# ytchen0323/cloud-scale-bwamem

Hardware: AMD Instinct MI355X
Metric: pair-end 2x150bp reads aligned/sec (higher is better)
Workload: dtype int32+u16

## Files before the change

### cloud-scale-bwamem_amd/csrc/bpsw_internal.h

```cpp
#pragma once

#include <hip/hip_runtime.h>
#include <stddef.h>
#include <stdint.h>

#include <condition_variable>
#include <cstdlib>
#include <mutex>
#include <string>
#include <vector>

#include "bpsw.h"
#include "bpsw_ext_group.h"
#include "bpsw_ring.h"

struct bpsw_ctx;

#include <hip/hip_ext.h>

namespace bpsw {

struct KernelEvents {
  hipEvent_t start = nullptr, stop = nullptr;
};
#define BPSW_LAUNCH(ev, kernel, grid, block, lds, stream, ...)                                                          \
  do {                                                                                                                   \
    if ((ev).start || (ev).stop) hipExtLaunchKernelGGL(kernel, grid, block, lds, stream, (ev).start, (ev).stop, 0, __VA_ARGS__); \
    else hipLaunchKernelGGL(kernel, grid, block, lds, stream, __VA_ARGS__);                                               \
  } while (0)


struct MatRows {
  unsigned long long row[5];
};
MatRows pack_mat(const int8_t mat[25]);
// ... 320 lines not shown
  std::mutex mu;
  DeviceBuffer buf;
  long long l_pac = 0;
  DeviceBuffer ann;
  std::vector<long long> ann_off;
  std::vector<int32_t> ann_len;
  std::vector<std::string> ann_name;
};
DeviceRef& device_ref(int device);

struct StreamLease {
  int device;
  hipStream_t s;
  bool pooled;
  bool led = false;
  int slot = -1;
  double wait_ms;
  explicit StreamLease(bpsw_ctx* c, ExtGroupWaiter* w = nullptr, ExtGroupWaiter** members = nullptr, int* n_members = nullptr);
  ~StreamLease();
  StreamLease(const StreamLease&) = delete;
  StreamLease& operator=(const StreamLease&) = delete;
};
struct CopyLane {
  std::mutex mu;
  hipStream_t s = nullptr;
  hipEvent_t ev = nullptr;
};
CopyLane& copy_lane(int device);
double wall_ms();
int ext_group_max();
int ext_group_waiting(int device);
void ext_group_counts(int device, unsigned long long out[3]);
void ext_group_complete(int device, ExtGroupWaiter** members, int n_members, int status, float span_ms);
void ext_call_mark(int device);
double ext_call_age_ms(int device);
double stat_ms();
int sw_launches_in_flight(int device);
void sw_launch_in_flight(int device, int delta);
double wait_est_update(double est, double took_ms, int polls, bool napped);
bool wait_naps(double est_ms);
void wait_nap(double est_ms);
void wait_poll_pause(int polls, double waited_ms, double est_ms);
hipError_t wait_event(bpsw_ctx* c, hipEvent_t ev, int kind);
int zerocopy_mask();
bool spin_wait();
[[nodiscard]] RefHold ref_snapshot(const bpsw_ctx* c, const uint8_t** pac, long long* l_pac);

int finish_pending_ext(bpsw_ctx* c);
int finish_pending_sw(bpsw_ctx* c);
inline int finish_pending(bpsw_ctx* c) {
  const int a = finish_pending_ext(c), b = finish_pending_sw(c);
  return a != BPSW_OK ? a : b;
}

int run_sw_jobs_host(bpsw_ctx* c, const bpsw_opt_t* opt, const bpsw_sw_jobs_t* jobs, int32_t* out);
struct SwStage {
  int n;
  size_t o_qlen, o_tlen, o_qoff, o_toff, o_qrev, o_qpool, o_tpool, o_packed, total, q_pool_bytes, t_pool_bytes;
  uint8_t* base;
};
int sw_stage_begin(bpsw_ctx* c, int n, size_t q_pool_bytes, size_t t_pool_bytes, SwStage* st);
int sw_stage_run(bpsw_ctx* c, const bpsw_opt_t* opt, int xtra, const SwStage& st, int mq, int mt, bool pac_mode, const int32_t** results);

struct ChainDevJob {
  int n_reads;
  const long long* seed_beg;
// ... 40 lines not shown
  bpsw::ExtScoring ext_sc;
  int8_t ext_mat[25];
  bpsw::DeviceBuffer d_wire, d_out, d_pre, d_sw_in, d_sw_out, d_sw_scratch, d_gl_z, d_ext_lists;
  size_t staged_bytes = 0;
  bpsw::DeviceBuffer d_sift;
  bpsw::DeviceBuffer d_seed[5];
  bpsw::DeviceBuffer d_chain;
  struct PendingExt { bool active = false; const void* d_wire = nullptr; size_t wire_bytes = 0; int n_tasks = 0; void* d_out = nullptr;
                      hipStream_t s = nullptr; int qcap = 0, rcap = 0; } pend_ext;
  int ext_geom_q = 0, ext_geom_r = 0;
  struct PendingSw { bool active = false; bpsw_sw_jobs_t jobs; bpsw_opt_t opt; void* d_out = nullptr; hipStream_t s = nullptr;
                     int cap_qlen = 0, cap_tlen = 0;
                     bool verified = false;
  } pend_sw;
  int sw_geom_qlen = 0, sw_geom_tlen = 0;
  float last_tail_ms = 0.f;
  int last_tail_jobs = 0, last_tail_resubmitted = 0;
  double tail_host_ms[3] = {0., 0., 0.};
  bool have_tail_ev = false;

  bpsw::PinnedBuffer h_stage_in, h_stage_out, h_pre;
  int shortcut_mask = 63;
  std::vector<int> ext_long_tasks;
  double wait_est_ms[6] = {0., 0., 0., 0., 0., 0.};
  bool ring_abandoned = false;
  uint32_t ring_seq = 0;
  void* rescue_scratch = nullptr;
  bpsw_stats_t stats;
  float last_ext_ms = 0.f, last_sw_ms = 0.f;
  bool have_ext_ev = false, have_sw_ev = false;
  bpsw::DeviceBuffer d_chain_tab;
};

namespace bpsw {
struct ContextEntry {
  std::unique_lock<std::mutex> lock;
  int rc = BPSW_OK;
  explicit ContextEntry(bpsw_ctx* c) : lock(c->mu) {
    if (c->ring_abandoned) { rc = fail(BPSW_ERR_DEVICE, "this context gave up a ring batch (watchdog / integrity): create a new one"); return; }
    const hipError_t e = hipSetDevice(c->device);
    if (e != hipSuccess) { rc = fail(BPSW_ERR_DEVICE, std::string("hipSetDevice: ") + hipGetErrorString(e)); return; }
    rc = finish_pending(c);
  }
};
}
```

### cloud-scale-bwamem_amd/csrc/bpsw_rescue.cpp

```cpp
#include <stdlib.h>
#include <string.h>

#include <algorithm>
#include <vector>

#include "bpsw_internal.h"
#include "bpsw_klib_sort.h"
#include "bpsw_rescue_skip.h"

using namespace bpsw;

namespace {

typedef bpsw_alnreg_t Reg;

struct LtRe {
  bool operator()(const Reg& x, const Reg& y) const { return x.re < y.re; }
};
struct LtScore {
  bool operator()(const Reg& x, const Reg& y) const {
    return x.score > y.score || (x.score == y.score && (x.rb < y.rb || (x.rb == y.rb && x.qb < y.qb)));
  }
};
struct LtReRb {
  bool operator()(const Reg& x, const Reg& y) const { return x.re < y.re || (x.re == y.re && x.rb < y.rb); }
};


int sort_dedup(std::vector<Reg>& v, float mask, int mode) {
  int n = (int)v.size();
// ... 12 lines not shown
      const int64_t mr = std::min(q.re - q.rb, p.re - p.rb);
      const int64_t mq = std::min<int64_t>(q.qe - q.qb, p.qe - p.qb);
      if ((float)orr > mask * (float)mr && (float)oq > mask * (float)mq) {
        if (p.score < q.score) { p.qe = p.qb; break; }
        q.qe = q.qb;
      }
    }
  }
  int m = 0;
  for (int i = 0; i < n; ++i)
    if (a[i].qe > a[i].qb) a[m++] = a[i];
  n = m;
  if (mode == BPSW_RESCUE_C) klib_order_sort((size_t)n, a, LtScore());
  else insertion_sort(a, a + n, LtScore());
  for (int i = 1; i < n; ++i)
    if (a[i].score == a[i - 1].score && a[i].rb == a[i - 1].rb && a[i].qb == a[i - 1].qb) a[i].qe = a[i].qb;
  m = n < 1 ? 0 : 1;
  for (int i = 1; i < n; ++i)
    if (a[i].qe > a[i].qb) a[m++] = a[i];
  v.resize((size_t)m);
  return m;
}

inline int infer_dir(int64_t l_pac, int64_t b1, int64_t b2, int64_t* dist) { return rescue_infer_dir(l_pac, b1, b2, dist); }

struct Want { int64_t x; int32_t mate; };
struct Scratch {
  std::vector<int64_t> t_base;
  std::vector<int64_t> job_x;
  std::vector<size_t> job_round;
  std::vector<int32_t> results;
  std::vector<uint8_t> used;
  std::vector<Want> want, want_next;
  std::vector<int32_t> touched;
  std::vector<int64_t> mate_slot;
  std::vector<int32_t> staged_mates;
  std::vector<Reg> arena;
  std::vector<int64_t> fin_off;
  std::vector<int32_t> fin_cnt;
  std::vector<uint8_t> done;
  std::vector<Reg> anchors[2], v[2];
};

struct Group {
  const bpsw_opt_t* opt;
  const bpsw_rescue_group_t* g;
  int mode;
  bool pac_mode;
  Scratch* S;
  int failed_mask;
  int32_t pes_low[4], pes_high[4];
};

void skip_flags(const Group& G, const Reg& a, const Reg* mates, size_t n_mates, int skip[4]) {
  rescue_skip_flags(G.g->l_pac, G.pes_low, G.pes_high, G.failed_mask, G.mode == BPSW_RESCUE_SCALA, a.rb, mates ? &mates->rb : nullptr, sizeof(Reg), n_mates, skip);
}

inline int64_t win_len(const Group& G, int64_t x) {
  if (!G.pac_mode) return G.g->ref_len[x];
  int64_t b = G.g->ref_rb[x], e = G.g->ref_re[x];
  if (b < 0 && e < 0) return 0;
  if (e < b) std::swap(b, e);
  if (e > (G.g->l_pac << 1)) e = G.g->l_pac << 1;
  if (b < 0) b = 0;
  if (!(b >= G.g->l_pac || e <= G.g->l_pac)) return 0;
  return e - b > 0 ? e - b : 0;
}
inline bool window_ok(const Group& G, int64_t x) { return win_len(G, x) == G.g->ref_re[x] - G.g->ref_rb[x]; }

bool make_region(const Group& G, const int32_t aln[7], int r, int l_ms, int64_t x, Reg* out) {
  if (!(aln[0] >= G.opt->min_seed_len && aln[6] >= 0)) return false;
  const bool is_rev = (r >> 1) != (r & 1);
  const int64_t l2 = G.g->l_pac << 1, rbeg = G.g->ref_rb[x];
  Reg b;
  memset(&b, 0, sizeof b);
  if (is_rev) {
    b.qb = l_ms - (aln[2] + 1); b.qe = l_ms - aln[6];
    b.rb = l2 - (rbeg + aln[1] + 1); b.re = l2 - (rbeg + aln[5]);
  } else {
    b.qb = aln[6]; b.qe = aln[2] + 1;
    if (G.mode == BPSW_RESCUE_C) { b.rb = rbeg + aln[5]; b.re = rbeg + aln[1] + 1; }
    else { b.rb = rbeg + aln[1] + 1; b.re = rbeg + aln[1] + 1; }
  }
  b.score = aln[0]; b.csub = aln[3]; b.secondary = -1;
  b.seedcov = (int32_t)(std::min<int64_t>(b.re - b.rb, b.qe - b.qb) >> 1);
  *out = b;
  return true;
}

static const int32_t kNoHit[7] = {0, -1, -1, -1, -1, -1, -1};
inline const int32_t* result_of(Group& G, int64_t x, int l_ms) {
// ... 96 lines not shown
                                 int32_t* out_cnt, bpsw_alnreg_t* out_regs, int64_t out_cap, int64_t* out_total) {
  if (!c || !opt || !g || !out_cnt || !out_total) return fail(BPSW_ERR_ARG, "matesw_group: null argument");
  if (mode != BPSW_RESCUE_C && mode != BPSW_RESCUE_SCALA) return fail(BPSW_ERR_ARG, "matesw_group: bad mode");
  const int G_ = g->group_size;
  if (G_ < 0) return fail(BPSW_ERR_ARG, "matesw_group: negative group size");
  ContextEntry entry(c);
  if (entry.rc != BPSW_OK) return entry.rc;

  const double t_begin = stat_ms();
  double t_pack = 0., t_replay = 0.;
  if (!c->rescue_scratch) c->rescue_scratch = new Scratch();
  Scratch& S = *(Scratch*)c->rescue_scratch;
  Group GR;
  GR.opt = opt; GR.g = g; GR.mode = mode; GR.S = &S;
  GR.pac_mode = g->ref_pool == nullptr;
  const bool rescue_on = (opt->flag & 0x20) == 0;

  GR.failed_mask = 0;
  for (int r = 0; r < 4; ++r) { GR.failed_mask |= (g->pes[r].failed ? 1 : 0) << r; GR.pes_low[r] = g->pes[r].low; GR.pes_high[r] = g->pes[r].high; }
  S.t_base.clear();
  S.want.clear(); S.touched.clear();
  int64_t nreg = 0, nref = 0;
  {
    const int32_t* reg_cnt = g->reg_cnt;
    const int32_t* ref_cnt = g->ref_cnt;
    const int32_t* seq_len = g->seq_len;
    const int64_t* seq_off = g->seq_off;
    const uint64_t pool_bytes = g->seq_pool_bytes;
    const int max_matesw = opt->max_matesw, pen_unpaired = opt->pen_unpaired;
    for (int k = 0; k < G_; ++k) {
      const int e0 = 2 * k;
      const int rc[2] = {reg_cnt[e0], reg_cnt[e0 + 1]}, fc[2] = {ref_cnt[e0], ref_cnt[e0 + 1]}, sl[2] = {seq_len[e0], seq_len[e0 + 1]};
      if ((rc[0] | rc[1] | fc[0] | fc[1] | sl[0] | sl[1]) < 0) return fail(BPSW_ERR_ARG, "matesw_group: negative count");
      if ((uint64_t)(seq_off[e0] + sl[0]) > pool_bytes || (uint64_t)(seq_off[e0 + 1] + sl[1]) > pool_bytes)
        return fail(BPSW_ERR_ARG, "matesw_group: mate outside seq_pool");
      const int64_t base[2] = {nreg, nreg + rc[0]}, rowb[2] = {nref, nref + fc[0]};
      nreg += (int64_t)rc[0] + rc[1]; nref += (int64_t)fc[0] + fc[1];
      if (!rescue_on) continue;
      __builtin_prefetch(g->regs + nreg + 12);
      __builtin_prefetch(g->regs + nreg + 13);
#ifndef BPSW_PLAN_PF_ROWS
#define BPSW_PLAN_PF_ROWS 16
#endif
      if (BPSW_PLAN_PF_ROWS > 0) {
        __builtin_prefetch(g->ref_rb + 4 * (nref + BPSW_PLAN_PF_ROWS));
        __builtin_prefetch(g->ref_re + 4 * (nref + BPSW_PLAN_PF_ROWS));
        if (!GR.pac_mode) __builtin_prefetch(g->ref_len + 4 * (nref + BPSW_PLAN_PF_ROWS));
      }
      if (rc[0] == 1 && rc[1] == 1 && fc[0] >= 1 && fc[1] >= 1 && sl[0] >= 1 && sl[1] >= 1 && max_matesw >= 1 && pen_unpaired >= 0) {
        const int64_t rb0 = g->regs[base[0]].rb, rb1 = g->regs[base[1]].rb;
        int64_t d01, d10;
        const int r01 = infer_dir(g->l_pac, rb0, rb1, &d01), r10 = infer_dir(g->l_pac, rb1, rb0, &d10);
        if (mode == BPSW_RESCUE_SCALA) { d01 = (int64_t)(int32_t)d01; d10 = (int64_t)(int32_t)d10; }
        const int m0 = GR.failed_mask | ((d01 >= GR.pes_low[r01] && d01 <= GR.pes_high[r01]) ? 1 << r01 : 0);
        const int m1 = GR.failed_mask | ((d10 >= GR.pes_low[r10] && d10 <= GR.pes_high[r10]) ? 1 << r10 : 0);
        if (m0 == 15 && m1 == 15) continue;
      }
      bool touched = false;
      for (int i = 0; i < 2; ++i) {
        const int mate = e0 + (i ^ 1);
        if (sl[i ^ 1] < 1 || rc[i] == 0 || fc[i] == 0) continue;
        const Reg* init = g->regs + base[i];
        const Reg* minit = g->regs + base[i ^ 1];
        const int n_init = rc[i], n_mate = rc[i ^ 1];
        const int thr = init[0].score - pen_unpaired;
        int j = 0;
        bool emitted = false;
        for (int ai = 0; ai < n_init; ++ai) {
          const Reg& a = init[ai];
          if (!(a.score >= thr)) continue;
          if (j >= max_matesw || j >= fc[i]) break;
          if (emitted) break;
          int skip[4];
          skip_flags(GR, a, minit, (size_t)n_mate, skip);
          if (skip[0] + skip[1] + skip[2] + skip[3] != 4) {
            const int64_t xrow = rowb[i] + j;
            for (int r = 0; r < 4; ++r)
              if (!skip[r] && window_ok(GR, xrow * 4 + r)) { S.want.push_back({xrow * 4 + r, mate}); touched = true; emitted = true; }
          }
          ++j;
        }
      }
      if (touched) {
        S.touched.push_back(k);
        S.t_base.push_back(base[0]); S.t_base.push_back(base[1]); S.t_base.push_back(rowb[0]); S.t_base.push_back(rowb[1]);
      }
    }
  }
  RefHold ref_hold;
  if (GR.pac_mode && nref > 0) {
    const uint8_t* d_pac = nullptr;
    long long loaded = 0;
    ref_hold = ref_snapshot(c, &d_pac, &loaded);
    if (loaded <= 0) return fail(BPSW_ERR_ARG, "matesw_group: ref_pool is null and no reference is loaded (bpsw_ref_load)");
    if (loaded != g->l_pac) return fail(BPSW_ERR_ARG, "matesw_group: l_pac differs from the loaded reference");
  }
  S.job_x.clear(); S.job_round.clear();
  S.results.clear(); S.used.clear();
  const double t_planned = stat_ms();

  const int xtra_base = BPSW_KSW_XSUBO | BPSW_KSW_XSTART | (opt->min_seed_len * opt->a);
  const size_t nt = S.touched.size();
  S.arena.clear();
  S.fin_off.assign(2 * nt, 0); S.fin_cnt.assign(2 * nt, 0); S.done.assign(nt, 0);
  S.mate_slot.assign(2 * (size_t)G_, (int64_t)-1);
  S.staged_mates.clear();
  uint64_t rounds = 0;
  const uint64_t speculated = S.want.size();
  size_t n_done = 0;
  for (;;) {
// ... 145 lines not shown
```

### cloud-scale-bwamem_amd/csrc/bpsw_runtime.cpp

```cpp
#include <stdlib.h>
#include <string.h>

#include <sched.h>
#include <time.h>

#include <algorithm>
#include <atomic>
#include <condition_variable>

#pragma weak launch_ext_group
#include "bpsw_internal.h"

namespace bpsw {

static thread_local std::string g_err;
void set_error(const std::string& msg) { g_err = msg; }
int fail(int code, const std::string& msg) {
  g_err = msg;
  return code;
}

struct RingPauseForFree {
  int dev = 0;
  RingPauseForFree() { if (hipGetDevice(&dev) != hipSuccess) dev = 0; ring_pause(dev); }
  ~RingPauseForFree() { ring_resume(dev); }
};

hipError_t DeviceBuffer::reserve(size_t bytes) {
  if (bytes <= cap) return hipSuccess;
  size_t want = cap ? cap : 1 << 20;
  while (want < bytes) want <<= 1;
  if (ptr) { RingPauseForFree paused; (void)hipFree(ptr); }
  ptr = nullptr;
  cap = 0;
// ... 128 lines not shown
int zerocopy_mask() {
  static const int m = getenv("BPSW_ZEROCOPY") ? atoi(getenv("BPSW_ZEROCOPY")) : 7;
  return m;
}

double wait_est_update(double est, double took_ms, int polls, bool napped) {
  (void)polls; (void)napped;
  if (est <= 0.) return took_ms;
  return 0.75 * est + 0.25 * std::min(took_ms, 3.0 * est + 0.2);
}
bool wait_naps(double est_ms) { return est_ms > 0.15 && est_ms * 700.0 - 60.0 > 20.0; }

void wait_nap(double est_ms) {
  if (est_ms > 0.15) {
    const double nap_us = est_ms * 700.0 - 60.0;
    if (nap_us > 20.0) { timespec ts = {0, (long)(nap_us * 1000.0)}; nanosleep(&ts, nullptr); }
  }
}
void wait_poll_pause(int polls, double waited_ms, double est_ms) {
  if (polls < 64 && waited_ms < est_ms * 1.3 + 0.05) sched_yield();
  else { timespec ts = {0, 20000}; nanosleep(&ts, nullptr); }
}

hipError_t wait_event(bpsw_ctx* c, hipEvent_t ev, int kind) {
  if (spin_wait()) return hipEventSynchronize(ev);
  double& est = c->wait_est_ms[kind & 3];
  const double t0 = wall_ms();
  const bool napped = wait_naps(est);
  wait_nap(est);
  hipError_t e;
  int polls = 0;
  while ((e = hipEventQuery(ev)) == hipErrorNotReady) wait_poll_pause(++polls, wall_ms() - t0, est);
  est = wait_est_update(est, wall_ms() - t0, polls, napped);
  return e;
}

double stat_ms() {
  static const bool cpu = getenv("BPSW_STATS_CLOCK") && getenv("BPSW_STATS_CLOCK")[0] == 'c';
  if (!cpu) return wall_ms();
  timespec ts;
  clock_gettime(CLOCK_THREAD_CPUTIME_ID, &ts);
  return 1e3 * (double)ts.tv_sec + 1e-6 * (double)ts.tv_nsec;
}

double wall_ms() {
  timespec ts;
  clock_gettime(CLOCK_MONOTONIC, &ts);
  return 1e3 * (double)ts.tv_sec + 1e-6 * (double)ts.tv_nsec;
}
// ... 27 lines not shown
  }();
  return cap;
}
int stream_share() {
  static const int n = [] {
    const char* e = getenv("BPSW_STREAM_SHARE");
    const int v = e ? atoi(e) : 1;
    return v < 1 ? 1 : (v > 8 ? 8 : v);
  }();
  return n;
}
}

static std::atomic<long long> g_ext_last_us[64];
void ext_call_mark(int device) { g_ext_last_us[device >= 0 && device < 64 ? device : 0].store((long long)(wall_ms() * 1e3), std::memory_order_relaxed); }
double ext_call_age_ms(int device) {
  const long long t = g_ext_last_us[device >= 0 && device < 64 ? device : 0].load(std::memory_order_relaxed);
  return t == 0 ? 1e12 : wall_ms() - (double)t * 1e-3;
}

CopyLane& copy_lane(int device) {
  static CopyLane table[64];
  return table[device >= 0 && device < 64 ? device : 0];
}

int ext_group_max() {
  static const int n = [] {
    const char* e = getenv("BPSW_EXT_GROUP_MAX");
    const int v = e ? atoi(e) : EXT_GROUP_SLOTS;
    return v < 1 ? 1 : (v > EXT_GROUP_SLOTS ? EXT_GROUP_SLOTS : v);
  }();
  return n;
}
int ext_group_waiting(int device) { return stream_pool(device).q.waiting_compatible(); }
void ext_group_counts(int device, unsigned long long out[3]) { stream_pool(device).q.counts(out); }
void ext_group_complete(int device, ExtGroupWaiter** members, int n_members, int status, float span_ms) {
  stream_pool(device).q.complete(members, n_members, status, span_ms);
}

static int pool_take(StreamPool& P, int cap) {
  if (P.streams.capacity() < 64) { P.streams.reserve(64); P.pending.reserve(64); }
  int best = -1;
  for (size_t k = 0; k < P.streams.size(); ++k)
    if (best < 0 || P.pending[k] < P.pending[(size_t)best]) best = (int)k;
  if (best >= 0 && P.pending[(size_t)best] == 0) { ++P.pending[(size_t)best]; return best; }
  if ((int)P.streams.size() < cap) {
// ... 155 lines not shown
  if (!c) return fail(BPSW_ERR_ARG, "null context");
  std::lock_guard<std::mutex> g(c->mu);
  c->shortcut_mask = mask < 0 ? 63 : (mask & 63);
  apply_shortcuts(c->shortcut_mask, c->ext_mat, &c->ext_sc.exact_a, &c->ext_sc.certify, &c->ext_sc.tail_bound);
  return BPSW_OK;
}

int bpsw_set_ext_scoring(bpsw_ctx_t* c, const int8_t mat[25], int zdrop, int zdrop_mode) {
  if (!c) return fail(BPSW_ERR_ARG, "null context");
  if (zdrop_mode != BPSW_ZDROP_SCALA && zdrop_mode != BPSW_ZDROP_BWA) return fail(BPSW_ERR_ARG, "bad zdrop_mode");
  std::lock_guard<std::mutex> g(c->mu);
  if (mat) memcpy(c->ext_mat, mat, 25);
  c->ext_sc.mat = pack_mat(c->ext_mat);
  c->ext_sc.mat_max = c->ext_mat[0];
  for (int k = 1; k < 25; ++k) c->ext_sc.mat_max = c->ext_mat[k] > c->ext_sc.mat_max ? c->ext_mat[k] : c->ext_sc.mat_max;
  c->ext_sc.zdrop = zdrop;
  c->ext_sc.zdrop_mode = zdrop_mode;
  apply_shortcuts(c->shortcut_mask, c->ext_mat, &c->ext_sc.exact_a, &c->ext_sc.certify, &c->ext_sc.tail_bound);
  return BPSW_OK;
}



static inline int rd16(const uint8_t* b, size_t at) { return (int16_t)(b[at] | (b[at + 1] << 8)); }
static inline int rd32(const uint8_t* b, size_t at) {
  return (int32_t)((uint32_t)b[at] | ((uint32_t)b[at + 1] << 8) | ((uint32_t)b[at + 2] << 16) | ((uint32_t)b[at + 3] << 24));
}

static int scan_wire(const uint8_t* wire, size_t bytes, long long l_pac, int* n_out, int* maxq, int* maxr, bool* coord,
                     std::vector<int>* long_tasks, int* maxr_short, int* n_mid_out) {
  if (!wire || bytes < 32 || (bytes & 3)) return fail(BPSW_ERR_ARG, "extend: wire batch shorter than its header or not word sized");
  const int n = rd32(wire, 8);
  const int fmt = wire[7];
  if (fmt != 0 && fmt != BPSW_WIRE_COORDS) return fail(BPSW_ERR_ARG, "extend: unknown wire format (header byte 7)");
  const bool co = fmt == BPSW_WIRE_COORDS;
  const size_t rec_bytes = co ? 40 : 32;
  if (n < 0 || 32 + rec_bytes * (size_t)n > bytes) return fail(BPSW_ERR_ARG, "extend: task table exceeds the buffer");
  if ((int8_t)wire[0] < 0 || (int8_t)wire[1] < 1 || (int8_t)wire[2] < 0 || (int8_t)wire[3] < 1)
    return fail(BPSW_ERR_ARG, "extend: gap opens must be >= 0 and gap extensions >= 1 (a zero extension divides by zero in SWUtil.scala:110-115)");
  if ((int8_t)wire[6] < 0) return fail(BPSW_ERR_ARG, "extend: negative band width (w travels as a signed byte: at most 127)");
  if (co && l_pac <= 0) return fail(BPSW_ERR_ARG, "extend: a coordinate batch needs the reference on the device (bpsw_ref_load)");
  const int wband = (int8_t)wire[6];
  int mq = 0, mr = 0, mrs = 0;
  const size_t words = bytes >> 2;
  const bool all_long = (int8_t)wire[2] + (int8_t)wire[3] <= 0;
  long_tasks->clear();
  int mid = 0;
  for (int t = 0; t < n; ++t) {
    const size_t at = 32 + rec_bytes * (size_t)t;
    const int lq = rd16(wire, at), lr = rd16(wire, at + 2), rq = rd16(wire, at + 4), rr = rd16(wire, at + 6);
    if (lq < 0 || lr < 0 || rq < 0 || rr < 0) return fail(BPSW_ERR_ARG, "extend: negative sequence length in task table");
    const long long pos = rd32(wire, at + 8);
    const long long w = co ? ((long long)lq + rq + 7) / 8 : ((long long)lq + lr + rq + rr + 7) / 8;
    if (pos < 8 + (long long)(rec_bytes / 4) * n || (unsigned long long)(pos + w) > words)
      return fail(BPSW_ERR_ARG, "extend: task sequence offset outside the buffer");
    if (lq > mq) mq = lq;
    if (rq > mq) mq = rq;
    const bool is_long = all_long || lq > 255 || rq > 255;
    const bool is_mid = !is_long && (lq > 127 || rq > 127);
    if (is_mid) ++mid;
    if (is_long) long_tasks->push_back(t);
    int task_mr = 0;
    if (co) {
      const int len = rd16(wire, at + 18);
      long long rb;
      memcpy(&rb, wire + at + 32, 8);
      if (rb < 0 || rb > (l_pac << 1)) return fail(BPSW_ERR_ARG, "extend: task window outside the reference or bridging its two strands");
      const long long lo = rb - lr, hi = rb + len + rr;
      if (len < 0 || lo < 0 || hi > (l_pac << 1) || (lo < l_pac && hi > l_pac))
        return fail(BPSW_ERR_ARG, "extend: task window outside the reference or bridging its two strands");
      const int sl = std::min(lr, lq + 2 * wband + 2), sr = std::min(rr, rq + 2 * wband + 2);
      task_mr = std::max(sl, sr);
    } else {
      task_mr = std::max(lr, rr);
    }
    if (task_mr > mr) mr = task_mr;
    if (!is_long && task_mr > mrs) mrs = task_mr;
  }
  if (mq > BPSW_EXT_MAX_QLEN || mr > BPSW_EXT_MAX_RLEN) return fail(BPSW_ERR_LIMIT, "extend: sequence longer than the kernel limit");
  *n_out = n; *maxq = mq; *maxr = mr; *coord = co; *maxr_short = mrs; *n_mid_out = mid;
  return BPSW_OK;
}

static int extend_batch_impl(bpsw_ctx_t* c, const uint8_t* wire, size_t wire_bytes, int16_t* out, size_t out_len, uint8_t* side_how,
                             const int16_t** out_view = nullptr);

int bpsw_extend_batch(bpsw_ctx_t* c, const uint8_t* wire, size_t wire_bytes, int16_t* out, size_t out_len) {
  return extend_batch_impl(c, wire, wire_bytes, out, out_len, nullptr);
}

int bpsw_extend_stage(bpsw_ctx_t* c, size_t bytes, uint8_t** buf) {
  if (!c || !buf) return fail(BPSW_ERR_ARG, "extend_stage: null argument");
  ContextEntry entry(c);
  if (entry.rc != BPSW_OK) return entry.rc;
  HIP_TRY(c->h_stage_in.reserve(bytes + bytes / 8 + 4096));
  c->staged_bytes = bytes;
  *buf = (uint8_t*)c->h_stage_in.ptr;
  return BPSW_OK;
}

int bpsw_extend_commit(bpsw_ctx_t* c, size_t wire_bytes, const int16_t** out, size_t* out_len) {
  if (!c || !out) return fail(BPSW_ERR_ARG, "extend_commit: null argument");
  const uint8_t* staged = nullptr;
// ... 114 lines not shown
                                   RingRecords{(uint32_t*)c->h_stage_out.ptr, 5, (size_t)n, 4, "extension"});
      if (run.how == RingRun::failed) {
        if (run.submitted) c->ring_abandoned = true;
        return run.rc;
      }
      if (run.how == RingRun::unwritten) {
        static std::atomic<bool> said{false};
        if (!said.exchange(true)) fprintf(stderr, "bPSW: an extension batch came back from the ring with unwritten records; it is run again through a launch (%s)\n", bpsw_last_error());
      }
      if (run.how == RingRun::done) {
        ring_kernel_ms = run.span_ms;
        t_dev1 = stat_ms();
        via_ring = true;
        c->stats.ext_ring_calls++;
      } else {
        copy_first_ms = 0.;
      }
    }
  }
  if (!via_ring) {
    const bool copy_first = sw_launches_in_flight(c->device) > 0;
    if (copy_first) {
      const double t_c0 = stat_ms();
      CopyLane& L = copy_lane(c->device);
      {
        std::lock_guard<std::mutex> lk(L.mu);
        if (!L.s) HIP_TRY(hipStreamCreateWithFlags(&L.s, hipStreamNonBlocking));
        HIP_TRY(hipMemcpyAsync(c->d_wire.ptr, c->h_stage_in.ptr, stage_bytes, hipMemcpyHostToDevice, L.s));
        HIP_TRY(hipStreamSynchronize(L.s));
      }
      copy_first_ms = stat_ms() - t_c0;
    }
    const bool zc_out = (zerocopy_mask() & 1) != 0;
    int16_t* k_out = zc_out ? (int16_t*)c->h_stage_out.ptr : (int16_t*)c->d_out.ptr;
    int* const d_queue_words = (int*)((char*)c->d_pre.ptr + 128);
    ExtCallItem me;
    memset(&me.gm, 0, sizeof me.gm);
    const bool groupable = &launch_ext_group != nullptr && ext_group_max() > 1 && !coord && use_sift && lazy_full && zc_out && !side_how;
    if (groupable) {
      ExtMember& m = me.gm.m;
      m.wire = (const uint32_t*)c->d_wire.ptr; m.n_tasks = n; m.out = k_out; m.sc = c->ext_sc; m.queue = d_queue_words;
      m.defer = (int*)((char*)c->d_wire.ptr + list_off); m.defer_post = (int*)(k_out + 10 * (size_t)n); m.short_qmax = 255;
      m.sift_flag = (uint8_t*)c->d_sift.ptr; m.sift_recs = (uint4*)((char*)c->d_sift.ptr + sift_rec_off);
      m.todo_count = d_queue_words + 2; m.todo_list = (int*)((char*)c->d_sift.ptr + todo_off);
      m.sift_dm = sift_dm; m.sift_dn = sift_uniform_dn(c->ext_mat, c->ext_sc.exact_a); m.sift_qmax = 127; m.heavy_min = heavy_min;
      me.gm.qcap = std::min(mq, 255); me.gm.rcap = mr_short;
      if (!copy_first) { me.copy_dst = c->d_wire.ptr; me.copy_src = c->h_stage_in.ptr; me.copy_bytes = stage_bytes; }
    }
    ExtGroupWaiter gw;
    gw.compatible = groupable;
    gw.item = &me;
    ExtGroupWaiter* led[EXT_GROUP_SLOTS];
    int n_led = 0;
// ... 280 lines not shown
```

Before: 265.7 million.

## Factor out rescue planning, branchless wire scan, and configurable copy-lane locking

```diff
diff --git a/cloud-scale-bwamem_amd/csrc/bpsw_copy_lane.h b/cloud-scale-bwamem_amd/csrc/bpsw_copy_lane.h
--- /dev/null
+++ b/cloud-scale-bwamem_amd/csrc/bpsw_copy_lane.h
@@ -0,0 +1,62 @@
+#pragma once
+#include <stddef.h>
+
+#include <mutex>
+
+namespace bpsw {
+
+enum CopyLaneMode { COPY_LANE_LOCK = 0, COPY_LANE_FIFO = 1, COPY_LANE_TWO = 2 };
+#ifndef COPY_LANE_DEFAULT
+#define COPY_LANE_DEFAULT COPY_LANE_LOCK
+#endif
+
+inline int copy_lane_mode_of(const char* s, int otherwise) {
+  if (!s) return otherwise;
+  if (s[0] == 'l') return COPY_LANE_LOCK;
+  if (s[0] == 'f') return COPY_LANE_FIFO;
+  if (s[0] == 't') return COPY_LANE_TWO;
+  return otherwise;
+}
+
+struct CopyLaneLocks {
+  std::mutex enqueue;
+  std::mutex head;
+};
+
+template <class Ops, class Wait>
+inline int copy_lane_copy(CopyLaneLocks& L, Ops& ops, int mode, void* dst, const void* src, size_t bytes, typename Ops::Event ev, Wait&& wait) {
+  if (mode == COPY_LANE_FIFO) {
+    {
+      std::lock_guard<std::mutex> lk(L.enqueue);
+      int rc = ops.enqueue_copy(dst, src, bytes);
+      if (rc == 0) rc = ops.record(ev);
+      if (rc != 0) return rc;
+    }
+    return wait(ev);
+  }
+  if (mode == COPY_LANE_TWO) {
+    std::unique_lock<std::mutex> first(L.enqueue);
+    int rc = ops.enqueue_copy(dst, src, bytes);
+    if (rc == 0) rc = ops.record(ev);
+    if (rc != 0) return rc;
+    std::lock_guard<std::mutex> second(L.head);
+    first.unlock();
+    return ops.synchronize(ev, false);
+  }
+  std::lock_guard<std::mutex> lk(L.enqueue);
+  const int rc = ops.enqueue_copy(dst, src, bytes);
+  if (rc != 0) return rc;
+  return ops.synchronize(ev, true);
+}
+
+template <class Ops, class Pause>
+inline int copy_lane_poll(Ops& ops, typename Ops::Event ev, Pause&& pause) {
+  for (;;) {
+    bool done = false;
+    const int rc = ops.query(ev, &done);
+    if (rc != 0 || done) return rc;
+    pause();
+  }
+}
+
+}
diff --git a/cloud-scale-bwamem_amd/csrc/bpsw_internal.h b/cloud-scale-bwamem_amd/csrc/bpsw_internal.h
--- a/cloud-scale-bwamem_amd/csrc/bpsw_internal.h
+++ b/cloud-scale-bwamem_amd/csrc/bpsw_internal.h
@@ -11,6 +11,7 @@
 #include <vector>
 
 #include "bpsw.h"
+#include "bpsw_copy_lane.h"
 #include "bpsw_ext_group.h"
 #include "bpsw_ring.h"
 
@@ -377,11 +378,12 @@
   StreamLease& operator=(const StreamLease&) = delete;
 };
 struct CopyLane {
-  std::mutex mu;
+  CopyLaneLocks locks;
   hipStream_t s = nullptr;
-  hipEvent_t ev = nullptr;
 };
 CopyLane& copy_lane(int device);
+int copy_lane_mode();
+hipError_t copy_lane_h2d(bpsw_ctx* c, void* dst, const void* src, size_t bytes);
 double wall_ms();
 int ext_group_max();
 int ext_group_waiting(int device);
@@ -397,6 +399,7 @@
 void wait_nap(double est_ms);
 void wait_poll_pause(int polls, double waited_ms, double est_ms);
 hipError_t wait_event(bpsw_ctx* c, hipEvent_t ev, int kind);
+hipError_t wait_event_est(hipEvent_t ev, double* est_ms);
 int zerocopy_mask();
 bool spin_wait();
 [[nodiscard]] RefHold ref_snapshot(const bpsw_ctx* c, const uint8_t** pac, long long* l_pac);
@@ -483,7 +486,7 @@
   bpsw::PinnedBuffer h_stage_in, h_stage_out, h_pre;
   int shortcut_mask = 63;
   std::vector<int> ext_long_tasks;
-  double wait_est_ms[6] = {0., 0., 0., 0., 0., 0.};
+  double wait_est_ms[7] = {0., 0., 0., 0., 0., 0., 0.};
   bool ring_abandoned = false;
   uint32_t ring_seq = 0;
   void* rescue_scratch = nullptr;
diff --git a/cloud-scale-bwamem_amd/csrc/bpsw_rescue.cpp b/cloud-scale-bwamem_amd/csrc/bpsw_rescue.cpp
--- a/cloud-scale-bwamem_amd/csrc/bpsw_rescue.cpp
+++ b/cloud-scale-bwamem_amd/csrc/bpsw_rescue.cpp
@@ -6,6 +6,7 @@
 
 #include "bpsw_internal.h"
 #include "bpsw_klib_sort.h"
+#include "bpsw_rescue_plan.h"
 #include "bpsw_rescue_skip.h"
 
 using namespace bpsw;
@@ -64,9 +65,7 @@
   return m;
 }
 
-inline int infer_dir(int64_t l_pac, int64_t b1, int64_t b2, int64_t* dist) { return rescue_infer_dir(l_pac, b1, b2, dist); }
-
-struct Want { int64_t x; int32_t mate; };
+typedef RescueWant Want;
 struct Scratch {
   std::vector<int64_t> t_base;
   std::vector<int64_t> job_x;
@@ -98,17 +97,8 @@
   rescue_skip_flags(G.g->l_pac, G.pes_low, G.pes_high, G.failed_mask, G.mode == BPSW_RESCUE_SCALA, a.rb, mates ? &mates->rb : nullptr, sizeof(Reg), n_mates, skip);
 }
 
-inline int64_t win_len(const Group& G, int64_t x) {
-  if (!G.pac_mode) return G.g->ref_len[x];
-  int64_t b = G.g->ref_rb[x], e = G.g->ref_re[x];
-  if (b < 0 && e < 0) return 0;
-  if (e < b) std::swap(b, e);
-  if (e > (G.g->l_pac << 1)) e = G.g->l_pac << 1;
-  if (b < 0) b = 0;
-  if (!(b >= G.g->l_pac || e <= G.g->l_pac)) return 0;
-  return e - b > 0 ? e - b : 0;
-}
-inline bool window_ok(const Group& G, int64_t x) { return win_len(G, x) == G.g->ref_re[x] - G.g->ref_rb[x]; }
+inline int64_t win_len(const Group& G, int64_t x) { return rescue_win_len(G.g, G.pac_mode, x); }
+inline bool window_ok(const Group& G, int64_t x) { return rescue_window_ok(G.g, G.pac_mode, x); }
 
 bool make_region(const Group& G, const int32_t aln[7], int r, int l_ms, int64_t x, Reg* out) {
   if (!(aln[0] >= G.opt->min_seed_len && aln[6] >= 0)) return false;
@@ -251,70 +241,14 @@
   S.want.clear(); S.touched.clear();
   int64_t nreg = 0, nref = 0;
   {
-    const int32_t* reg_cnt = g->reg_cnt;
-    const int32_t* ref_cnt = g->ref_cnt;
-    const int32_t* seq_len = g->seq_len;
-    const int64_t* seq_off = g->seq_off;
-    const uint64_t pool_bytes = g->seq_pool_bytes;
-    const int max_matesw = opt->max_matesw, pen_unpaired = opt->pen_unpaired;
-    for (int k = 0; k < G_; ++k) {
-      const int e0 = 2 * k;
-      const int rc[2] = {reg_cnt[e0], reg_cnt[e0 + 1]}, fc[2] = {ref_cnt[e0], ref_cnt[e0 + 1]}, sl[2] = {seq_len[e0], seq_len[e0 + 1]};
-      if ((rc[0] | rc[1] | fc[0] | fc[1] | sl[0] | sl[1]) < 0) return fail(BPSW_ERR_ARG, "matesw_group: negative count");
-      if ((uint64_t)(seq_off[e0] + sl[0]) > pool_bytes || (uint64_t)(seq_off[e0 + 1] + sl[1]) > pool_bytes)
-        return fail(BPSW_ERR_ARG, "matesw_group: mate outside seq_pool");
-      const int64_t base[2] = {nreg, nreg + rc[0]}, rowb[2] = {nref, nref + fc[0]};
-      nreg += (int64_t)rc[0] + rc[1]; nref += (int64_t)fc[0] + fc[1];
-      if (!rescue_on) continue;
-      __builtin_prefetch(g->regs + nreg + 12);
-      __builtin_prefetch(g->regs + nreg + 13);
-#ifndef BPSW_PLAN_PF_ROWS
-#define BPSW_PLAN_PF_ROWS 16
-#endif
-      if (BPSW_PLAN_PF_ROWS > 0) {
-        __builtin_prefetch(g->ref_rb + 4 * (nref + BPSW_PLAN_PF_ROWS));
-        __builtin_prefetch(g->ref_re + 4 * (nref + BPSW_PLAN_PF_ROWS));
-        if (!GR.pac_mode) __builtin_prefetch(g->ref_len + 4 * (nref + BPSW_PLAN_PF_ROWS));
-      }
-      if (rc[0] == 1 && rc[1] == 1 && fc[0] >= 1 && fc[1] >= 1 && sl[0] >= 1 && sl[1] >= 1 && max_matesw >= 1 && pen_unpaired >= 0) {
-        const int64_t rb0 = g->regs[base[0]].rb, rb1 = g->regs[base[1]].rb;
-        int64_t d01, d10;
-        const int r01 = infer_dir(g->l_pac, rb0, rb1, &d01), r10 = infer_dir(g->l_pac, rb1, rb0, &d10);
-        if (mode == BPSW_RESCUE_SCALA) { d01 = (int64_t)(int32_t)d01; d10 = (int64_t)(int32_t)d10; }
-        const int m0 = GR.failed_mask | ((d01 >= GR.pes_low[r01] && d01 <= GR.pes_high[r01]) ? 1 << r01 : 0);
-        const int m1 = GR.failed_mask | ((d10 >= GR.pes_low[r10] && d10 <= GR.pes_high[r10]) ? 1 << r10 : 0);
-        if (m0 == 15 && m1 == 15) continue;
-      }
-      bool touched = false;
-      for (int i = 0; i < 2; ++i) {
-        const int mate = e0 + (i ^ 1);
-        if (sl[i ^ 1] < 1 || rc[i] == 0 || fc[i] == 0) continue;
-        const Reg* init = g->regs + base[i];
-        const Reg* minit = g->regs + base[i ^ 1];
-        const int n_init = rc[i], n_mate = rc[i ^ 1];
-        const int thr = init[0].score - pen_unpaired;
-        int j = 0;
-        bool emitted = false;
-        for (int ai = 0; ai < n_init; ++ai) {
-          const Reg& a = init[ai];
-          if (!(a.score >= thr)) continue;
-          if (j >= max_matesw || j >= fc[i]) break;
-          if (emitted) break;
-          int skip[4];
-          skip_flags(GR, a, minit, (size_t)n_mate, skip);
-          if (skip[0] + skip[1] + skip[2] + skip[3] != 4) {
-            const int64_t xrow = rowb[i] + j;
-            for (int r = 0; r < 4; ++r)
-              if (!skip[r] && window_ok(GR, xrow * 4 + r)) { S.want.push_back({xrow * 4 + r, mate}); touched = true; emitted = true; }
-          }
-          ++j;
-        }
-      }
-      if (touched) {
-        S.touched.push_back(k);
-        S.t_base.push_back(base[0]); S.t_base.push_back(base[1]); S.t_base.push_back(rowb[0]); S.t_base.push_back(rowb[1]);
-      }
-    }
+    RescuePlanCfg cfg;
+    cfg.failed_mask = GR.failed_mask;
+    for (int r = 0; r < 4; ++r) { cfg.low[r] = GR.pes_low[r]; cfg.high[r] = GR.pes_high[r]; }
+    cfg.scala = mode == BPSW_RESCUE_SCALA; cfg.pac_mode = GR.pac_mode; cfg.rescue_on = rescue_on;
+    cfg.max_matesw = opt->max_matesw; cfg.pen_unpaired = opt->pen_unpaired;
+    const int prc = rescue_plan(g, cfg, S.want, S.touched, S.t_base, &nreg, &nref);
+    if (prc == RESCUE_PLAN_NEGATIVE_COUNT) return fail(BPSW_ERR_ARG, "matesw_group: negative count");
+    if (prc != RESCUE_PLAN_OK) return fail(BPSW_ERR_ARG, "matesw_group: mate outside seq_pool");
   }
   RefHold ref_hold;
   if (GR.pac_mode && nref > 0) {
diff --git a/cloud-scale-bwamem_amd/csrc/bpsw_rescue_plan.h b/cloud-scale-bwamem_amd/csrc/bpsw_rescue_plan.h
--- /dev/null
+++ b/cloud-scale-bwamem_amd/csrc/bpsw_rescue_plan.h
@@ -0,0 +1,128 @@
+#pragma once
+#include <stdint.h>
+
+#include <utility>
+#include <vector>
+
+#include "bpsw.h"
+#include "bpsw_rescue_skip.h"
+
+namespace bpsw {
+
+struct RescueWant { int64_t x; int32_t mate; };
+
+struct RescuePlanCfg {
+  int failed_mask;
+  int32_t low[4], high[4];
+  bool scala;
+  bool pac_mode;
+  bool rescue_on;
+  int max_matesw, pen_unpaired;
+};
+
+enum { RESCUE_PLAN_OK = 0, RESCUE_PLAN_NEGATIVE_COUNT = 1, RESCUE_PLAN_MATE_OUTSIDE = 2 };
+
+#ifndef RESCUE_PLAN_AHEAD
+#define RESCUE_PLAN_AHEAD 32
+#endif
+
+inline int64_t rescue_win_len(const bpsw_rescue_group_t* g, bool pac_mode, int64_t x) {
+  if (!pac_mode) return g->ref_len[x];
+  int64_t b = g->ref_rb[x], e = g->ref_re[x];
+  if (b < 0 && e < 0) return 0;
+  if (e < b) std::swap(b, e);
+  if (e > (g->l_pac << 1)) e = g->l_pac << 1;
+  if (b < 0) b = 0;
+  if (!(b >= g->l_pac || e <= g->l_pac)) return 0;
+  return e - b > 0 ? e - b : 0;
+}
+inline bool rescue_window_ok(const bpsw_rescue_group_t* g, bool pac_mode, int64_t x) {
+  return rescue_win_len(g, pac_mode, x) == g->ref_re[x] - g->ref_rb[x];
+}
+
+inline void rescue_plan_prefetch(const void* base, int64_t at, size_t elem_bytes) {
+  __builtin_prefetch((const void*)((uintptr_t)base + (uintptr_t)at * elem_bytes));
+}
+
+inline bool rescue_plan_all_skipped(int64_t l_pac, const RescuePlanCfg& cfg, int64_t a_rb, int64_t m_rb) {
+  int64_t d;
+  const int r = rescue_infer_dir(l_pac, a_rb, m_rb, &d);
+  if (cfg.scala) d = (int64_t)(int32_t)d;
+  const int in = (int)(d >= cfg.low[r]) & (int)(d <= cfg.high[r]);
+  return (cfg.failed_mask | (in << r)) == 15;
+}
+
+inline void rescue_plan_walk_pair(const bpsw_rescue_group_t* g, const RescuePlanCfg& cfg, int k, int64_t base0, int64_t rowb0,
+                                  std::vector<RescueWant>& want, std::vector<int32_t>& touched_pairs, std::vector<int64_t>& t_base) {
+  const int e0 = 2 * k;
+  const int rc[2] = {g->reg_cnt[e0], g->reg_cnt[e0 + 1]}, fc[2] = {g->ref_cnt[e0], g->ref_cnt[e0 + 1]}, sl[2] = {g->seq_len[e0], g->seq_len[e0 + 1]};
+  const int64_t base[2] = {base0, base0 + rc[0]}, rowb[2] = {rowb0, rowb0 + fc[0]};
+  bool touched = false;
+  for (int i = 0; i < 2; ++i) {
+    const int mate = e0 + (i ^ 1);
+    if (sl[i ^ 1] < 1 || rc[i] == 0 || fc[i] == 0) continue;
+    const bpsw_alnreg_t* init = g->regs + base[i];
+    const bpsw_alnreg_t* minit = g->regs + base[i ^ 1];
+    const int n_init = rc[i], n_mate = rc[i ^ 1];
+    const int thr = init[0].score - cfg.pen_unpaired;
+    int j = 0;
+    bool emitted = false;
+    for (int ai = 0; ai < n_init; ++ai) {
+      const bpsw_alnreg_t& a = init[ai];
+      if (!(a.score >= thr)) continue;
+      if (j >= cfg.max_matesw || j >= fc[i]) break;
+      if (emitted) break;
+      int skip[4];
+      rescue_skip_flags(g->l_pac, cfg.low, cfg.high, cfg.failed_mask, cfg.scala, a.rb, n_mate ? &minit->rb : nullptr, sizeof(bpsw_alnreg_t),
+                        (size_t)n_mate, skip);
+      if (skip[0] + skip[1] + skip[2] + skip[3] != 4) {
+        const int64_t xrow = rowb[i] + j;
+        for (int r = 0; r < 4; ++r)
+          if (!skip[r] && rescue_window_ok(g, cfg.pac_mode, xrow * 4 + r)) { want.push_back({xrow * 4 + r, mate}); touched = true; emitted = true; }
+      }
+      ++j;
+    }
+  }
+  if (touched) {
+    touched_pairs.push_back(k);
+    t_base.push_back(base[0]); t_base.push_back(base[1]); t_base.push_back(rowb[0]); t_base.push_back(rowb[1]);
+  }
+}
+
+inline int rescue_plan(const bpsw_rescue_group_t* g, const RescuePlanCfg& cfg, std::vector<RescueWant>& want, std::vector<int32_t>& touched,
+                       std::vector<int64_t>& t_base, int64_t* nreg_out, int64_t* nref_out) {
+  const int G = g->group_size;
+  const int32_t* reg_cnt = g->reg_cnt;
+  const int32_t* ref_cnt = g->ref_cnt;
+  const int32_t* seq_len = g->seq_len;
+  const int64_t* seq_off = g->seq_off;
+  const bpsw_alnreg_t* regs = g->regs;
+  const uint64_t pool_bytes = g->seq_pool_bytes;
+  const int64_t l_pac = g->l_pac;
+  const bool fast_shape = cfg.max_matesw >= 1 && cfg.pen_unpaired >= 0;
+  int64_t nreg = 0, nref = 0;
+  int err = RESCUE_PLAN_OK;
+  for (int k = 0; k < G; ++k) {
+    const int e0 = 2 * k;
+    const int rc0 = reg_cnt[e0], rc1 = reg_cnt[e0 + 1], fc0 = ref_cnt[e0], fc1 = ref_cnt[e0 + 1], sl0 = seq_len[e0], sl1 = seq_len[e0 + 1];
+    if ((rc0 | rc1 | fc0 | fc1 | sl0 | sl1) < 0) { err = RESCUE_PLAN_NEGATIVE_COUNT; break; }
+    if ((uint64_t)(seq_off[e0] + sl0) > pool_bytes || (uint64_t)(seq_off[e0 + 1] + sl1) > pool_bytes) { err = RESCUE_PLAN_MATE_OUTSIDE; break; }
+    const int64_t base0 = nreg, rowb0 = nref;
+    nreg += (int64_t)rc0 + rc1; nref += (int64_t)fc0 + fc1;
+    if (!cfg.rescue_on) continue;
+    rescue_plan_prefetch(regs, nreg + RESCUE_PLAN_AHEAD, sizeof *regs);
+    rescue_plan_prefetch(regs, nreg + RESCUE_PLAN_AHEAD + 1, sizeof *regs);
+    rescue_plan_prefetch(g->ref_rb, 4 * (nref + RESCUE_PLAN_AHEAD), 8);
+    rescue_plan_prefetch(g->ref_re, 4 * (nref + RESCUE_PLAN_AHEAD), 8);
+    if (!cfg.pac_mode) rescue_plan_prefetch(g->ref_len, 4 * (nref + RESCUE_PLAN_AHEAD), 8);
+    if (fast_shape & (rc0 == 1) & (rc1 == 1) & (fc0 >= 1) & (fc1 >= 1) & (sl0 >= 1) & (sl1 >= 1)) {
+      const int64_t rb0 = regs[base0].rb, rb1 = regs[base0 + 1].rb;
+      if ((int)rescue_plan_all_skipped(l_pac, cfg, rb0, rb1) & (int)rescue_plan_all_skipped(l_pac, cfg, rb1, rb0)) continue;
+    }
+    rescue_plan_walk_pair(g, cfg, k, base0, rowb0, want, touched, t_base);
+  }
+  *nreg_out = nreg; *nref_out = nref;
+  return err;
+}
+
+}
diff --git a/cloud-scale-bwamem_amd/csrc/bpsw_runtime.cpp b/cloud-scale-bwamem_amd/csrc/bpsw_runtime.cpp
--- a/cloud-scale-bwamem_amd/csrc/bpsw_runtime.cpp
+++ b/cloud-scale-bwamem_amd/csrc/bpsw_runtime.cpp
@@ -10,6 +10,7 @@
 
 #pragma weak launch_ext_group
 #include "bpsw_internal.h"
+#include "bpsw_wire_scan.h"
 
 namespace bpsw {
 
@@ -184,9 +185,11 @@
   else { timespec ts = {0, 20000}; nanosleep(&ts, nullptr); }
 }
 
-hipError_t wait_event(bpsw_ctx* c, hipEvent_t ev, int kind) {
+hipError_t wait_event(bpsw_ctx* c, hipEvent_t ev, int kind) { return wait_event_est(ev, &c->wait_est_ms[kind & 3]); }
+
+hipError_t wait_event_est(hipEvent_t ev, double* est_ms) {
   if (spin_wait()) return hipEventSynchronize(ev);
-  double& est = c->wait_est_ms[kind & 3];
+  double& est = *est_ms;
   const double t0 = wall_ms();
   const bool napped = wait_naps(est);
   wait_nap(est);
@@ -260,6 +263,33 @@
 CopyLane& copy_lane(int device) {
   static CopyLane table[64];
   return table[device >= 0 && device < 64 ? device : 0];
+}
+int copy_lane_mode() {
+  static const int mode = copy_lane_mode_of(getenv("BPSW_COPY_LANE"), COPY_LANE_DEFAULT);
+  return mode;
+}
+namespace {
+struct HipLaneOps {
+  typedef hipEvent_t Event;
+  hipStream_t* s;
+  int enqueue_copy(void* dst, const void* src, size_t bytes) {
+    if (!*s) { const hipError_t e = hipStreamCreateWithFlags(s, hipStreamNonBlocking); if (e != hipSuccess) return (int)e; }
+    return (int)hipMemcpyAsync(dst, src, bytes, hipMemcpyHostToDevice, *s);
+  }
+  int record(Event ev) { return (int)hipEventRecord(ev, *s); }
+  int query(Event ev, bool* done) {
+    const hipError_t e = hipEventQuery(ev);
+    *done = e == hipSuccess;
+    return e == hipErrorNotReady ? 0 : (int)e;
+  }
+  int synchronize(Event ev, bool whole_stream) { return (int)(whole_stream ? hipStreamSynchronize(*s) : hipEventSynchronize(ev)); }
+};
+}
+hipError_t copy_lane_h2d(bpsw_ctx* c, void* dst, const void* src, size_t bytes) {
+  CopyLane& L = copy_lane(c->device);
+  HipLaneOps ops{&L.s};
+  double* est = &c->wait_est_ms[6];
+  return (hipError_t)copy_lane_copy(L.locks, ops, copy_lane_mode(), dst, src, bytes, c->ev[0], [est](hipEvent_t ev) { return (int)wait_event_est(ev, est); });
 }
 
 int ext_group_max() {
@@ -461,63 +491,15 @@
 
 
 
-static inline int rd16(const uint8_t* b, size_t at) { return (int16_t)(b[at] | (b[at + 1] << 8)); }
-static inline int rd32(const uint8_t* b, size_t at) {
-  return (int32_t)((uint32_t)b[at] | ((uint32_t)b[at + 1] << 8) | ((uint32_t)b[at + 2] << 16) | ((uint32_t)b[at + 3] << 24));
-}
+static inline int rd32(const uint8_t* b, size_t at) { return wire_rd32(b, at); }
 
 static int scan_wire(const uint8_t* wire, size_t bytes, long long l_pac, int* n_out, int* maxq, int* maxr, bool* coord,
                      std::vector<int>* long_tasks, int* maxr_short, int* n_mid_out) {
-  if (!wire || bytes < 32 || (bytes & 3)) return fail(BPSW_ERR_ARG, "extend: wire batch shorter than its header or not word sized");
-  const int n = rd32(wire, 8);
-  const int fmt = wire[7];
-  if (fmt != 0 && fmt != BPSW_WIRE_COORDS) return fail(BPSW_ERR_ARG, "extend: unknown wire format (header byte 7)");
-  const bool co = fmt == BPSW_WIRE_COORDS;
-  const size_t rec_bytes = co ? 40 : 32;
-  if (n < 0 || 32 + rec_bytes * (size_t)n > bytes) return fail(BPSW_ERR_ARG, "extend: task table exceeds the buffer");
-  if ((int8_t)wire[0] < 0 || (int8_t)wire[1] < 1 || (int8_t)wire[2] < 0 || (int8_t)wire[3] < 1)
-    return fail(BPSW_ERR_ARG, "extend: gap opens must be >= 0 and gap extensions >= 1 (a zero extension divides by zero in SWUtil.scala:110-115)");
-  if ((int8_t)wire[6] < 0) return fail(BPSW_ERR_ARG, "extend: negative band width (w travels as a signed byte: at most 127)");
-  if (co && l_pac <= 0) return fail(BPSW_ERR_ARG, "extend: a coordinate batch needs the reference on the device (bpsw_ref_load)");
-  const int wband = (int8_t)wire[6];
-  int mq = 0, mr = 0, mrs = 0;
-  const size_t words = bytes >> 2;
-  const bool all_long = (int8_t)wire[2] + (int8_t)wire[3] <= 0;
-  long_tasks->clear();
-  int mid = 0;
-  for (int t = 0; t < n; ++t) {
-    const size_t at = 32 + rec_bytes * (size_t)t;
-    const int lq = rd16(wire, at), lr = rd16(wire, at + 2), rq = rd16(wire, at + 4), rr = rd16(wire, at + 6);
-    if (lq < 0 || lr < 0 || rq < 0 || rr < 0) return fail(BPSW_ERR_ARG, "extend: negative sequence length in task table");
-    const long long pos = rd32(wire, at + 8);
-    const long long w = co ? ((long long)lq + rq + 7) / 8 : ((long long)lq + lr + rq + rr + 7) / 8;
-    if (pos < 8 + (long long)(rec_bytes / 4) * n || (unsigned long long)(pos + w) > words)
-      return fail(BPSW_ERR_ARG, "extend: task sequence offset outside the buffer");
-    if (lq > mq) mq = lq;
-    if (rq > mq) mq = rq;
-    const bool is_long = all_long || lq > 255 || rq > 255;
-    const bool is_mid = !is_long && (lq > 127 || rq > 127);
-    if (is_mid) ++mid;
-    if (is_long) long_tasks->push_back(t);
-    int task_mr = 0;
-    if (co) {
-      const int len = rd16(wire, at + 18);
-      long long rb;
-      memcpy(&rb, wire + at + 32, 8);
-      if (rb < 0 || rb > (l_pac << 1)) return fail(BPSW_ERR_ARG, "extend: task window outside the reference or bridging its two strands");
-      const long long lo = rb - lr, hi = rb + len + rr;
-      if (len < 0 || lo < 0 || hi > (l_pac << 1) || (lo < l_pac && hi > l_pac))
-        return fail(BPSW_ERR_ARG, "extend: task window outside the reference or bridging its two strands");
-      const int sl = std::min(lr, lq + 2 * wband + 2), sr = std::min(rr, rq + 2 * wband + 2);
-      task_mr = std::max(sl, sr);
-    } else {
-      task_mr = std::max(lr, rr);
-    }
-    if (task_mr > mr) mr = task_mr;
-    if (!is_long && task_mr > mrs) mrs = task_mr;
-  }
-  if (mq > BPSW_EXT_MAX_QLEN || mr > BPSW_EXT_MAX_RLEN) return fail(BPSW_ERR_LIMIT, "extend: sequence longer than the kernel limit");
-  *n_out = n; *maxq = mq; *maxr = mr; *coord = co; *maxr_short = mrs; *n_mid_out = mid;
+  WireScan ws;
+  const char* msg = nullptr;
+  const int rc = wire_scan(wire, bytes, l_pac, &ws, long_tasks, &msg);
+  if (rc != BPSW_OK) return fail(rc, msg);
+  *n_out = ws.n; *maxq = ws.maxq; *maxr = ws.maxr; *coord = ws.coord; *maxr_short = ws.maxr_short; *n_mid_out = ws.n_mid;
   return BPSW_OK;
 }
 
@@ -678,13 +660,7 @@
     const bool copy_first = sw_launches_in_flight(c->device) > 0;
     if (copy_first) {
       const double t_c0 = stat_ms();
-      CopyLane& L = copy_lane(c->device);
-      {
-        std::lock_guard<std::mutex> lk(L.mu);
-        if (!L.s) HIP_TRY(hipStreamCreateWithFlags(&L.s, hipStreamNonBlocking));
-        HIP_TRY(hipMemcpyAsync(c->d_wire.ptr, c->h_stage_in.ptr, stage_bytes, hipMemcpyHostToDevice, L.s));
-        HIP_TRY(hipStreamSynchronize(L.s));
-      }
+      HIP_TRY(copy_lane_h2d(c, c->d_wire.ptr, c->h_stage_in.ptr, stage_bytes));
       copy_first_ms = stat_ms() - t_c0;
     }
     const bool zc_out = (zerocopy_mask() & 1) != 0;
diff --git a/cloud-scale-bwamem_amd/csrc/bpsw_wire_scan.h b/cloud-scale-bwamem_amd/csrc/bpsw_wire_scan.h
--- /dev/null
+++ b/cloud-scale-bwamem_amd/csrc/bpsw_wire_scan.h
@@ -0,0 +1,141 @@
+#pragma once
+#include <stdint.h>
+#include <string.h>
+
+#include <algorithm>
+#include <vector>
+
+#include "bpsw.h"
+
+namespace bpsw {
+
+inline int wire_rd16(const uint8_t* b, size_t at) { return (int16_t)(b[at] | (b[at + 1] << 8)); }
+inline int wire_rd32(const uint8_t* b, size_t at) {
+  return (int32_t)((uint32_t)b[at] | ((uint32_t)b[at + 1] << 8) | ((uint32_t)b[at + 2] << 16) | ((uint32_t)b[at + 3] << 24));
+}
+
+struct WireScan {
+  int n = 0, maxq = 0, maxr = 0;
+  bool coord = false;
+  int maxr_short = 0;
+  int n_mid = 0;
+};
+
+#define BPSW_WIRE_MSG_NEG "extend: negative sequence length in task table"
+#define BPSW_WIRE_MSG_POS "extend: task sequence offset outside the buffer"
+#define BPSW_WIRE_MSG_WIN "extend: task window outside the reference or bridging its two strands"
+
+inline const char* wire_scan_refusal(const uint8_t* wire, size_t words, int n, bool co, long long l_pac) {
+  const size_t rec_bytes = co ? 40 : 32;
+  for (int t = 0; t < n; ++t) {
+    const size_t at = 32 + rec_bytes * (size_t)t;
+    const int lq = wire_rd16(wire, at), lr = wire_rd16(wire, at + 2), rq = wire_rd16(wire, at + 4), rr = wire_rd16(wire, at + 6);
+    if (lq < 0 || lr < 0 || rq < 0 || rr < 0) return BPSW_WIRE_MSG_NEG;
+    const long long pos = wire_rd32(wire, at + 8);
+    const long long w = co ? ((long long)lq + rq + 7) / 8 : ((long long)lq + lr + rq + rr + 7) / 8;
+    if (pos < 8 + (long long)(rec_bytes / 4) * n || (unsigned long long)(pos + w) > words) return BPSW_WIRE_MSG_POS;
+    if (co) {
+      const int len = wire_rd16(wire, at + 18);
+      long long rb;
+      memcpy(&rb, wire + at + 32, 8);
+      if (rb < 0 || rb > (l_pac << 1)) return BPSW_WIRE_MSG_WIN;
+      const long long lo = rb - lr, hi = rb + len + rr;
+      if (len < 0 || lo < 0 || hi > (l_pac << 1) || (lo < l_pac && hi > l_pac)) return BPSW_WIRE_MSG_WIN;
+    }
+  }
+  return nullptr;
+}
+
+struct WireSweep { int mq = 0, mr = 0, mrs = 0, mid = 0, n_long = 0; bool bad = false; };
+
+template <bool CO>
+inline WireSweep wire_sweep(const uint8_t* wire, size_t words, int n, bool all_long, int wband, long long l_pac) {
+  const size_t rec_bytes = CO ? 40 : 32;
+  const long long min_pos = 8 + (long long)(rec_bytes / 4) * n;
+  const long long l2 = l_pac << 1;
+  WireSweep s;
+  int bad = 0;
+  const int every = all_long ? 1 : 0;
+  for (int t = 0; t < n; ++t) {
+    const uint8_t* rec = wire + 32 + rec_bytes * (size_t)t;
+    struct { int16_t lq, lr, rq, rr; int32_t pos; } h;
+    memcpy(&h, rec, 12);
+    const int lq = h.lq, lr = h.lr, rq = h.rq, rr = h.rr;
+    const long long pos = h.pos;
+    bad |= (int)((lq | lr | rq | rr) < 0);
+    const long long w = (CO ? lq + rq + 7 : lq + lr + rq + rr + 7) >> 3;
+    bad |= (int)(pos < min_pos) | (int)((unsigned long long)(pos + w) > words);
+    s.mq = std::max(s.mq, std::max(lq, rq));
+    const int is_long = every | (int)(lq > 255) | (int)(rq > 255);
+    s.n_long += is_long;
+    s.mid += (is_long ^ 1) & ((int)(lq > 127) | (int)(rq > 127));
+    int task_mr;
+    if (CO) {
+      int16_t len16;
+      long long rb;
+      memcpy(&len16, rec + 18, 2);
+      memcpy(&rb, rec + 32, 8);
+      const int len = len16;
+      const int rb_bad = (int)(rb < 0) | (int)(rb > l2);
+      const long long rbs = rb_bad ? 0 : rb;
+      const long long lo = rbs - lr, hi = rbs + len + rr;
+      bad |= rb_bad | (int)(len < 0) | (int)(lo < 0) | (int)(hi > l2) | ((int)(lo < l_pac) & (int)(hi > l_pac));
+      const int sl = std::min(lr, lq + 2 * wband + 2), sr = std::min(rr, rq + 2 * wband + 2);
+      task_mr = std::max(sl, sr);
+    } else {
+      task_mr = std::max(lr, rr);
+    }
+    s.mr = std::max(s.mr, task_mr);
+    s.mrs = std::max(s.mrs, is_long ? 0 : task_mr);
+  }
+  s.bad = bad != 0;
+  return s;
+}
+
+inline int wire_scan(const uint8_t* wire, size_t bytes, long long l_pac, WireScan* out, std::vector<int>* long_tasks, const char** msg) {
+  *msg = nullptr;
+  if (!wire || bytes < 32 || (bytes & 3)) { *msg = "extend: wire batch shorter than its header or not word sized"; return BPSW_ERR_ARG; }
+  const int n = wire_rd32(wire, 8);
+  const int fmt = wire[7];
+  if (fmt != 0 && fmt != BPSW_WIRE_COORDS) { *msg = "extend: unknown wire format (header byte 7)"; return BPSW_ERR_ARG; }
+  const bool co = fmt == BPSW_WIRE_COORDS;
+  const size_t rec_bytes = co ? 40 : 32;
+  if (n < 0 || 32 + rec_bytes * (size_t)n > bytes) { *msg = "extend: task table exceeds the buffer"; return BPSW_ERR_ARG; }
+  if ((int8_t)wire[0] < 0 || (int8_t)wire[1] < 1 || (int8_t)wire[2] < 0 || (int8_t)wire[3] < 1) {
+    *msg = "extend: gap opens must be >= 0 and gap extensions >= 1 (a zero extension divides by zero in SWUtil.scala:110-115)";
+    return BPSW_ERR_ARG;
+  }
+  if ((int8_t)wire[6] < 0) { *msg = "extend: negative band width (w travels as a signed byte: at most 127)"; return BPSW_ERR_ARG; }
+  if (co && l_pac <= 0) { *msg = "extend: a coordinate batch needs the reference on the device (bpsw_ref_load)"; return BPSW_ERR_ARG; }
+  const int wband = (int8_t)wire[6];
+  const size_t words = bytes >> 2;
+  const bool all_long = (int8_t)wire[2] + (int8_t)wire[3] <= 0;
+  long_tasks->clear();
+  const WireSweep s = co ? wire_sweep<true>(wire, words, n, all_long, wband, l_pac) : wire_sweep<false>(wire, words, n, all_long, wband, l_pac);
+  if (s.bad) {
+    *msg = wire_scan_refusal(wire, words, n, co, l_pac);
+    if (!*msg) *msg = "extend: malformed task table";
+    return BPSW_ERR_ARG;
+  }
+  if (s.n_long) {
+    long_tasks->resize((size_t)s.n_long);
+    int* list = long_tasks->data();
+    int at = 0;
+    if (all_long) {
+      for (int t = 0; t < n; ++t) list[t] = t;
+    } else {
+      for (int t = 0; t < n && at < s.n_long; ++t) {
+        const uint8_t* rec = wire + 32 + rec_bytes * (size_t)t;
+        int16_t lq, rq;
+        memcpy(&lq, rec, 2);
+        memcpy(&rq, rec + 4, 2);
+        if (lq > 255 || rq > 255) list[at++] = t;
+      }
+    }
+  }
+  if (s.mq > BPSW_EXT_MAX_QLEN || s.mr > BPSW_EXT_MAX_RLEN) { *msg = "extend: sequence longer than the kernel limit"; return BPSW_ERR_LIMIT; }
+  out->n = n; out->maxq = s.mq; out->maxr = s.mr; out->coord = co; out->maxr_short = s.mrs; out->n_mid = s.mid;
+  return BPSW_OK;
+}
+
+}
```

New measurement: 258.8 million. 0.974x the previous value.
